# graphdeco-inria/hierarchical-3d-gaussians

Hardware: AMD Instinct MI355X
Metric: fwd+bwd frames/s @1080p, 1M Gaussians (higher is better)
Workload: dtype f32

## Files before the change

### hierarchical-3d-gaussians_amd/csrc/preprocess.hip

```cpp
#include "gaussian_math.h"

#include <stdlib.h>

#include <mutex>

namespace hgs {

namespace {

struct CamLds {
  float vm[16];
  float pm[16];
  float cam[3];
};

__device__ __forceinline__ void load_camera(const hgs_raster_args& a, CamLds& c) {
#pragma unroll
  for (int i = 0; i < 16; ++i) {
    c.vm[i] = a.viewmatrix[i];
    c.pm[i] = a.projmatrix[i];
  }
  c.cam[0] = a.campos[0];
  c.cam[1] = a.campos[1];
  c.cam[2] = a.campos[2];
// ... 747 lines not shown
}

constexpr int kPresumGrid = 2048;
__global__ __launch_bounds__(kPreBlock) void k8_presum_work_kernel(const uint2* __restrict__ work,
                                                                   const uint32_t* __restrict__ counter,
                                                                   const uint32_t* __restrict__ tiles_touched,
                                                                   const uint32_t* __restrict__ offsets,
                                                                   float* __restrict__ inst) {
  __shared__ double red_all[kPreBlock / 64][640 + 40];
  const int lane = threadIdx.x & 63, wave = threadIdx.x >> 6;
  const uint32_t n_work = *counter;
  double* red = red_all[wave];
  for (uint32_t item = blockIdx.x * (kPreBlock / 64) + wave; item < n_work; item += gridDim.x * (kPreBlock / 64)) {
    const uint2 w = work[item];
    const uint32_t n = tiles_touched[w.x];
    const uint32_t r0 = w.y * kK8Seg;
    const uint32_t r1 = (w.y + 1u == k8_nseg(n)) ? n : r0 + kK8Seg;
    const size_t rbase = (size_t)offsets[w.x] + r0;
    const float2* ip = reinterpret_cast<const float2*>(inst) + rbase * 5;
    double t[10];
#pragma unroll
    for (int i = 0; i < 10; ++i) t[i] = 0.0;
#pragma unroll 4
    for (uint32_t k = (uint32_t)lane; k < r1 - r0; k += 64u) {
      const float2 v0 = ip[k * 5 + 0], v1 = ip[k * 5 + 1], v2 = ip[k * 5 + 2], v3 = ip[k * 5 + 3], v4 = ip[k * 5 + 4];
      t[0] += v0.x; t[1] += v0.y; t[2] += v1.x; t[3] += v1.y;
      t[4] += v2.x; t[5] += v2.y; t[6] += v3.x; t[7] += v3.y;
      t[8] += v4.x; t[9] += v4.y;
    }
#pragma unroll
    for (int i = 0; i < 10; ++i) red[i * 64 + lane] = t[i];
    __builtin_amdgcn_fence(__ATOMIC_RELEASE, "wavefront");
    __builtin_amdgcn_wave_barrier();
    __builtin_amdgcn_fence(__ATOMIC_ACQUIRE, "wavefront");
    if (lane < 40) {
      double acc = 0.0;
      const double* src = red + (lane >> 2) * 64 + (lane & 3) * 16;
#pragma unroll
      for (int j = 0; j < 16; ++j) acc += src[j];
      red[640 + lane] = acc;
    }
    __builtin_amdgcn_fence(__ATOMIC_RELEASE, "wavefront");
    __builtin_amdgcn_wave_barrier();
    __builtin_amdgcn_fence(__ATOMIC_ACQUIRE, "wavefront");
    if (lane < 10) {
      const double* q = red + 640 + lane * 4;
      reinterpret_cast<double*>(inst + rbase * kInstStride)[lane] = ((q[0] + q[1]) + q[2]) + q[3];
    }
    __builtin_amdgcn_fence(__ATOMIC_RELEASE, "wavefront");
    __builtin_amdgcn_wave_barrier();
  }
}

template <bool ACC, bool LOD>
__global__ __launch_bounds__(kPreBlock) void preprocess_bwd_kernel(hgs_raster_args a, GeomWs g,
                                                                   const float* __restrict__ inst,
                                                                   float* __restrict__ drgb,
                                                                   float* __restrict__ dmean_rows,
                                                                   const uint32_t* __restrict__ lod_flag,
                                                                   hgs_raster_grads out, int presummed) {
  const int idx = blockIdx.x * kPreBlock + threadIdx.x;
  const bool in_range = idx < a.P;
  const uint32_t n = in_range ? g.tiles_touched[idx] : 0u;

  double s[10];
#pragma unroll
  for (int i = 0; i < 10; ++i) s[i] = 0.0;
  static_assert(kInstStride == 10, "instance record = the ten sums, 40 bytes");
  {
    constexpr uint32_t kStageRec = 256;
    __shared__ float2 stage[kPreBlock / 64][kStageRec * 5];
    const int lane = threadIdx.x & 63, wave = threadIdx.x >> 6;
    const unsigned long long long_mask = presummed ? __ballot(n > kK8LongRun) : 0ull;
    if (long_mask == 0ull) {
      uint32_t incl = n;
#pragma unroll
      for (int off = 1; off < 64; off <<= 1) {
        const uint32_t t = __shfl_up(incl, off, 64);
        if (lane >= off) incl += t;
      }
      const uint32_t my0 = incl - n, my1 = incl;
      const uint32_t total = __shfl(incl, 63, 64);
      if (total) {
        const unsigned long long nz = __ballot(n != 0u);
        const int first = __ffsll((long long)nz) - 1;
        const uint32_t off_mine = n ? g.offsets[idx] : 0u;
        const size_t base = (size_t)__shfl(off_mine, first, 64);
        float2* st = stage[wave];
        for (uint32_t c0 = 0; c0 < total; c0 += kStageRec) {
          const uint32_t cn = min(kStageRec, total - c0) * 5u;
          const float2* src = reinterpret_cast<const float2*>(inst) + (base + c0) * 5;
          for (uint32_t t0 = 0; t0 < cn; t0 += 64u * 4u) {
            float2 v[4];
#pragma unroll
            for (int j = 0; j < 4; ++j) {
              const uint32_t t = t0 + (uint32_t)j * 64u + (uint32_t)lane;
              v[j] = src[min(t, cn - 1u)];
            }
#pragma unroll
            for (int j = 0; j < 4; ++j) {
              const uint32_t t = t0 + (uint32_t)j * 64u + (uint32_t)lane;
              if (t < cn) st[t] = v[j];
            }
          }
          __builtin_amdgcn_fence(__ATOMIC_RELEASE, "wavefront");
          __builtin_amdgcn_wave_barrier();
          __builtin_amdgcn_fence(__ATOMIC_ACQUIRE, "wavefront");
          const uint32_t k0 = max(my0, c0), k1 = min(my1, c0 + kStageRec);
          for (uint32_t k = k0; k < k1; ++k) {
            const float2* r = st + (k - c0) * 5u;
            const float2 v0 = r[0], v1 = r[1], v2 = r[2], v3 = r[3], v4 = r[4];
            s[0] += v0.x; s[1] += v0.y; s[2] += v1.x; s[3] += v1.y;
            s[4] += v2.x; s[5] += v2.y; s[6] += v3.x; s[7] += v3.y;
            s[8] += v4.x; s[9] += v4.y;
          }
          __builtin_amdgcn_fence(__ATOMIC_RELEASE, "wavefront");
          __builtin_amdgcn_wave_barrier();
        }
      }
    } else if (n != 0u) {
      const size_t off = (size_t)g.offsets[idx];
      if (n > kK8LongRun) {
        const uint32_t nseg = k8_nseg(n);
        for (uint32_t j = 0; j < nseg; ++j) {
          const double* ps = reinterpret_cast<const double*>(inst + (off + (size_t)j * kK8Seg) * kInstStride);
#pragma unroll
          for (int i = 0; i < 10; ++i) s[i] += ps[i];
        }
      } else {
        const float2* ip = reinterpret_cast<const float2*>(inst) + off * 5;
#pragma unroll 2
        for (uint32_t k = 0; k < n; ++k) {
          const float2 v0 = ip[k * 5 + 0], v1 = ip[k * 5 + 1], v2 = ip[k * 5 + 2], v3 = ip[k * 5 + 3], v4 = ip[k * 5 + 4];
          s[0] += v0.x; s[1] += v0.y; s[2] += v1.x; s[3] += v1.y;
          s[4] += v2.x; s[5] += v2.y; s[6] += v3.x; s[7] += v3.y;
          s[8] += v4.x; s[9] += v4.y;
        }
      }
    }
  }
  if constexpr (!LOD) {
    if (!in_range) return;
  }

  float d_mean[3] = {0.f, 0.f, 0.f};
  float d_m2[3] = {0.f, 0.f, 0.f};
  float d_op = 0.f;
  float d_scale[3] = {0.f, 0.f, 0.f};
  float d_rot[4] = {0.f, 0.f, 0.f, 0.f};
  float d_c3[6] = {0.f, 0.f, 0.f, 0.f, 0.f, 0.f};
  float d_col[3] = {0.f, 0.f, 0.f};
  float sums6 = 0.f, sums7 = 0.f, sums8 = 0.f;

  if (n == 0) {
  } else {
    CamLds cam;
    load_camera(a, cam);
    sums6 = (float)s[6]; sums7 = (float)s[7]; sums8 = (float)s[8];
    const uint32_t flags = g.flags[idx];
    float p[3];
    load_mean<LOD>(a, lod_row_gather<LOD>(a, idx), p);
    float q[4] = {1.f, 0.f, 0.f, 0.f};
    float sc[3] = {1.f, 1.f, 1.f};
    double qnorm = 1.0;
    ProjD pd;
    if (a.cov3D_precomp) {
#pragma unroll
      for (int i = 0; i < 6; ++i) pd.c3[i] = (double)a.cov3D_precomp[(size_t)idx * 6 + i];
    } else {
      load_scale_rot<LOD>(a, idx, sc, q, &qnorm);
      cov3d_from_scale_rot_d(sc, a.scale_modifier, q, pd);
    }
    project_gaussian_d(p, cam.vm, cam.pm, a.width, a.height, a.tanfovx, a.tanfovy, (flags & 8u) != 0,
                       (flags & 16u) != 0, pd);

    const double A = pd.conA, B = pd.conB, C = pd.conC;
    const double gA = -0.5 * s[2], gB = -s[3], gC = -0.5 * s[4];
    const double ggx = -(A * s[0] + B * s[1]);
    const double ggy = -(C * s[1] + B * s[0]);
    const double dm2x = ggx * 0.5 * (double)a.width, dm2y = ggy * 0.5 * (double)a.height;
    d_m2[0] = (float)dm2x;
    d_m2[1] = (float)dm2y;
    double dmean[3] = {0.0, 0.0, 0.0};

    const double dhx = dm2x * pd.pw, dhy = dm2y * pd.pw;
    const double dhw = -(dm2x * pd.hx + dm2y * pd.hy) * pd.pw * pd.pw;
#pragma unroll
    for (int j = 0; j < 3; ++j)
      dmean[j] += (double)cam.pm[j * 4 + 0] * dhx + (double)cam.pm[j * 4 + 1] * dhy + (double)cam.pm[j * 4 + 3] * dhw;

    const double a2 = pd.a, b2 = pd.b, c2 = pd.c;
    const double di2 = pd.di * pd.di;
    const double ga = (-c2 * c2 * gA + b2 * c2 * gB - b2 * b2 * gC) * di2;
    const double gb = (2.0 * b2 * c2 * gA - (a2 * c2 + b2 * b2) * gB + 2.0 * a2 * b2 * gC) * di2;
    const double gc = (-b2 * b2 * gA + a2 * b2 * gB - a2 * a2 * gC) * di2;
    const double hb = 0.5 * gb;
    double Gs[3][3];
#pragma unroll
    for (int i = 0; i < 3; ++i)
#pragma unroll
      for (int j = i; j < 3; ++j)
        Gs[i][j] = Gs[j][i] = pd.T0[i] * (ga * pd.T0[j] + hb * pd.T1[j]) + pd.T1[i] * (hb * pd.T0[j] + gc * pd.T1[j]);
    d_c3[0] = (float)Gs[0][0];
    d_c3[1] = (float)(2.0 * Gs[0][1]);
    d_c3[2] = (float)(2.0 * Gs[0][2]);
    d_c3[3] = (float)Gs[1][1];
    d_c3[4] = (float)(2.0 * Gs[1][2]);
    d_c3[5] = (float)Gs[2][2];
    double dT0[3], dT1[3];
#pragma unroll
    for (int j = 0; j < 3; ++j) {
      dT0[j] = 2.0 * ga * pd.U0[j] + gb * pd.U1[j];
      dT1[j] = gb * pd.U0[j] + 2.0 * gc * pd.U1[j];
    }
    double gJ00 = 0.0, gJ02 = 0.0, gJ11 = 0.0, gJ12 = 0.0;
#pragma unroll
    for (int j = 0; j < 3; ++j) {
      gJ00 += dT0[j] * (double)cam.vm[j * 4 + 0];
      gJ02 += dT0[j] * (double)cam.vm[j * 4 + 2];
      gJ11 += dT1[j] * (double)cam.vm[j * 4 + 1];
      gJ12 += dT1[j] * (double)cam.vm[j * 4 + 2];
    }
    const double itz = pd.itz, itz2 = itz * itz, itz3 = itz2 * itz;
    const double g_txc = -pd.fx * itz2 * gJ02;
    const double g_tyc = -pd.fy * itz2 * gJ12;
    double g_tz = -pd.fx * itz2 * gJ00 + 2.0 * pd.fx * pd.txc * itz3 * gJ02 - pd.fy * itz2 * gJ11 +
                  2.0 * pd.fy * pd.tyc * itz3 * gJ12;
    double g_tx = 0.0, g_ty = 0.0;
    if (flags & 8u) g_tz += g_txc * (pd.txc * itz); else g_tx = g_txc;
    if (flags & 16u) g_tz += g_tyc * (pd.tyc * itz); else g_ty = g_tyc;
    g_tz += -s[9] * itz2;
#pragma unroll
    for (int j = 0; j < 3; ++j)
      dmean[j] += (double)cam.vm[j * 4 + 0] * g_tx + (double)cam.vm[j * 4 + 1] * g_ty + (double)cam.vm[j * 4 + 2] * g_tz;
    d_mean[0] = (float)dmean[0]; d_mean[1] = (float)dmean[1]; d_mean[2] = (float)dmean[2];

    if (!a.cov3D_precomp) {
      const double* R = pd.R;
      const double* sv = pd.s;
      double dM[3][3];
#pragma unroll
      for (int i = 0; i < 3; ++i)
#pragma unroll
        for (int k = 0; k < 3; ++k) {
          double acc = 0.0;
#pragma unroll
          for (int j = 0; j < 3; ++j) acc += Gs[i][j] * (R[j * 3 + k] * sv[k]);
          dM[i][k] = 2.0 * acc;
        }
      double gR[3][3];
#pragma unroll
      for (int k = 0; k < 3; ++k) {
        double acc = 0.0;
#pragma unroll
        for (int i = 0; i < 3; ++i) {
          acc += R[i * 3 + k] * dM[i][k];
          gR[i][k] = dM[i][k] * sv[k];
        }
        double dsk = (double)a.scale_modifier * acc;
        if (a.activations & HGS_ACT_SCALE_EXP) dsk *= (double)sc[k];
        d_scale[k] = (float)dsk;
      }
      const double r = q[0], x = q[1], y = q[2], z = q[3];
      double dq[4];
      dq[0] = 2.0 * (-z * gR[0][1] + y * gR[0][2] + z * gR[1][0] - x * gR[1][2] - y * gR[2][0] + x * gR[2][1]);
      dq[1] = 2.0 * (y * gR[0][1] + z * gR[0][2] + y * gR[1][0] - 2.0 * x * gR[1][1] - r * gR[1][2] +
                     z * gR[2][0] + r * gR[2][1] - 2.0 * x * gR[2][2]);
      dq[2] = 2.0 * (-2.0 * y * gR[0][0] + x * gR[0][1] + r * gR[0][2] + x * gR[1][0] + z * gR[1][2] -
                     r * gR[2][0] + z * gR[2][1] - 2.0 * y * gR[2][2]);
      dq[3] = 2.0 * (-2.0 * z * gR[0][0] - r * gR[0][1] + x * gR[0][2] + r * gR[1][0] - 2.0 * z * gR[1][1] +
                     y * gR[1][2] + x * gR[2][0] + y * gR[2][1]);
      if (a.activations & HGS_ACT_ROT_NORMALIZE) {
        const double dot = r * dq[0] + x * dq[1] + y * dq[2] + z * dq[3];
        const double inv = 1.0 / qnorm;
        dq[0] = (dq[0] - r * dot) * inv; dq[1] = (dq[1] - x * dot) * inv;
        dq[2] = (dq[2] - y * dot) * inv; dq[3] = (dq[3] - z * dot) * inv;
      }
      d_rot[0] = (float)dq[0]; d_rot[1] = (float)dq[1]; d_rot[2] = (float)dq[2]; d_rot[3] = (float)dq[3];
    }

    {
      float dod = 1.0f;
      double dact = 1.0;
      const float o_act = load_opacity<LOD>(a, idx, &dact);
      float o_rec = o_act;
      if (a.interpolation_weights && a.num_node_kids && !a.lod_per_pixel)
        o_rec = lod_opacity(o_act, a.interpolation_weights[idx], a.num_node_kids[idx], &dod);
      const float sums5 = o_rec > 0.0f ? (float)(s[5] / (double)o_rec) : 0.0f;
      d_op = a.activations ? (float)((double)sums5 * (double)dod * dact) : sums5 * dod;
    }

    float gr[3] = {sums6, sums7, sums8};
    if (a.colors_precomp) {
      d_col[0] = gr[0]; d_col[1] = gr[1]; d_col[2] = gr[2];
    } else {
      if (flags & 1u) gr[0] = 0.f;
      if (flags & 2u) gr[1] = 0.f;
      if (flags & 4u) gr[2] = 0.f;
      drgb[idx * 3 + 0] = gr[0];
      drgb[idx * 3 + 1] = gr[1];
      drgb[idx * 3 + 2] = gr[2];
    }
  }

  if constexpr (LOD) {
    if (a.lod_scatter) {
      __shared__ float lds_v[8 * kPreBlock];
      __shared__ int lds_par[kPreBlock];
      __shared__ unsigned char lds_vis[kPreBlock];
      const int t = threadIdx.x;
      const int block_first = blockIdx.x * kPreBlock;
      const int count = min(kPreBlock, a.P - block_first);
      LodRow l;
      l.r = l.p = 0; l.w = 1.0f; l.u = 0.0f;
      if (in_range) l = lod_row<true>(a, idx);
      const bool self = l.p == l.r;
      const bool vis = in_range && n != 0;
      const float wn = self ? 1.0f : l.w, u = (self || !vis) ? 0.0f : l.u;
      float sgn = 1.0f;
      if (vis && !self && u != 0.0f) {
        const float4 qa = reinterpret_cast<const float4*>(a.rotations)[l.r];
        const float4 qb = reinterpret_cast<const float4*>(a.rotations)[l.p];
        sgn = (qa.x * qb.x + qa.y * qb.y + qa.z * qb.z + qa.w * qb.w) < 0.0f ? -1.0f : 1.0f;
      }
      if (in_range) {
#pragma unroll
        for (int j = 0; j < 3; ++j) {
          dmean_rows[idx * 3 + j] = d_mean[j];
          out.dL_dmeans2D[idx * 3 + j] = d_m2[j];
        }
      }
      if (vis) {
        out.dL_dopacity[l.r] = wn * d_op;
#pragma unroll
        for (int j = 0; j < 3; ++j) out.dL_dscales[l.r * 3 + j] = wn * d_scale[j];
        reinterpret_cast<float4*>(out.dL_drotations)[l.r] = make_float4(wn * d_rot[0], wn * d_rot[1], wn * d_rot[2], wn * d_rot[3]);
      }
      lds_par[t] = in_range ? (int)l.p : -1;
      lds_vis[t] = (vis && !self) ? 1 : 0;
#pragma unroll
      for (int j = 0; j < 3; ++j) lds_v[j * kPreBlock + t] = u * d_scale[j];
#pragma unroll
      for (int j = 0; j < 4; ++j) lds_v[(3 + j) * kPreBlock + t] = (u * sgn) * d_rot[j];
      lds_v[7 * kPreBlock + t] = u * d_op;
      __syncthreads();
      if (t < count) {
        const LodRun run = lod_run(a, lds_par, t, count, block_first, *lod_flag != 0u);
        if (run.leader) {
          float acc8[8] = {0.f, 0.f, 0.f, 0.f, 0.f, 0.f, 0.f, 0.f};
          bool any = false;
          for (int j = t; j < run.end; ++j) {
            if (!lds_vis[j]) continue;
            any = true;
#pragma unroll
            for (int k = 0; k < 8; ++k) acc8[k] += lds_v[k * kPreBlock + j];
          }
          if (any) {
            const size_t pp = (size_t)lds_par[t];
#pragma unroll
            for (int k = 0; k < 3; ++k) lod_add(out.dL_dscales + pp * 3 + k, acc8[k], run.atomic);
#pragma unroll
            for (int k = 0; k < 4; ++k) lod_add(out.dL_drotations + pp * 4 + k, acc8[3 + k], run.atomic);
            lod_add(out.dL_dopacity + pp, acc8[7], run.atomic);
          }
        }
      }
      return;
    }
    if (!in_range) return;
  }
  constexpr bool acc = ACC;
#pragma unroll
  for (int j = 0; j < 3; ++j) {
    out.dL_dmeans3D[idx * 3 + j] = d_mean[j] + (acc ? out.dL_dmeans3D[idx * 3 + j] : 0.f);
    out.dL_dmeans2D[idx * 3 + j] = d_m2[j];
  }
  out.dL_dopacity[idx] = d_op + (acc ? out.dL_dopacity[idx] : 0.f);
  if (out.dL_dcolors) {
#pragma unroll
    for (int j = 0; j < 3; ++j) out.dL_dcolors[idx * 3 + j] = d_col[j];
  }
  if (out.dL_dscales) {
#pragma unroll
    for (int j = 0; j < 3; ++j) out.dL_dscales[idx * 3 + j] = d_scale[j] + (acc ? out.dL_dscales[idx * 3 + j] : 0.f);
  }
  if (out.dL_drotations) {
    float4* dst = reinterpret_cast<float4*>(out.dL_drotations) + idx;
    float4 v = make_float4(d_rot[0], d_rot[1], d_rot[2], d_rot[3]);
    if (acc) { const float4 o = *dst; v.x += o.x; v.y += o.y; v.z += o.z; v.w += o.w; }
    *dst = v;
  }
  if (out.dL_dcov3D) {
#pragma unroll
    for (int j = 0; j < 6; ++j) out.dL_dcov3D[(size_t)idx * 6 + j] = d_c3[j] + (acc ? out.dL_dcov3D[(size_t)idx * 6 + j] : 0.f);
  }
}


template <bool ACC, bool JAC, bool LOD>
__global__ __launch_bounds__(kPreBlock) void sh_bwd_kernel(hgs_raster_args a, GeomWs g,
                                                           const float* __restrict__ drgb,
                                                           const float* __restrict__ dmean_rows,
                                                           const uint32_t* __restrict__ lod_flag, hgs_raster_grads out) {
  extern __shared__ __attribute__((aligned(16))) unsigned char smem_raw[];
  float* lds = reinterpret_cast<float*>(smem_raw);
  const int n = a.M * 3;
  const bool split = a.shs_rest != nullptr;
  const bool coop = (n & 3) == 0;
  const int block_first = blockIdx.x * kPreBlock;
  const int idx = block_first + threadIdx.x;
  const bool valid = idx < a.P;
  const bool active = valid && g.tiles_touched[idx] != 0;
  if (!JAC && coop) {
    if (split) {
      coop_load_seg(a.shs, block_first, a.P, 3, 0, sh_row_stride(n), lds);
      coop_load_seg(a.shs_rest, block_first, a.P, n - 3, 3, sh_row_stride(n), lds);
    } else {
      coop_load_sh(a.shs, block_first, a.P, n, lds);
    }
    __syncthreads();
  }
  float dsh[48];
#pragma unroll
  for (int i = 0; i < 48; ++i) dsh[i] = 0.f;
  float sh[JAC ? 1 : 48];
  if constexpr (!JAC) {
    if (active) {
      if (coop) lds_row_read(lds, n, sh);
      else if (split) load_sh_split(a.shs, a.shs_rest, idx, a.M, sh);
      else load_sh(a.shs, idx, a.M, sh);
    }
  }
  if (!JAC && coop) __syncthreads();
  float vdir[3] = {0.f, 0.f, 0.f};
  if (active) {
    const float gr[3] = {drgb[idx * 3 + 0], drgb[idx * 3 + 1], drgb[idx * 3 + 2]};
    float pm[3];
    load_mean<LOD>(a, lod_row_gather<LOD>(a, idx), pm);
    float ux, uy, uz;
    const float inv = unit_dir(pm, a.campos, ux, uy, uz);
    float b[16];
    sh_basis(a.sh_degree, ux, uy, uz, b);
    const int nb = (a.sh_degree + 1) * (a.sh_degree + 1);
    float gdx = 0.f, gdy = 0.f, gdz = 0.f;
    if constexpr (JAC) {
      const float* jp = g.shjac + (size_t)idx * kJacStride;
      float J[9];
#pragma unroll
// ... 87 lines not shown
          const float wn = self ? 1.0f : rp[n + 2];
#pragma unroll
          for (int j = 0; j < 3; ++j) out.dL_dmeans3D[(size_t)r * 3 + j] = wn * lds_m[j * kPreBlock + t];
        }
        const LodRun run = lod_run(a, lds_par, t, count, block_first, nonmono);
        if (run.leader) {
          float acc3[3] = {0.f, 0.f, 0.f};
          bool any = false;
          for (int j = t; j < run.end; ++j) {
            const float* rj = lds + j * stride;
            if (!__float_as_uint(rj[n + 3]) || __float_as_uint(rj[n]) == __float_as_uint(rj[n + 1])) continue;
            any = true;
            const float uj = 1.0f - rj[n + 2];
#pragma unroll
            for (int k = 0; k < 3; ++k) acc3[k] += uj * lds_m[k * kPreBlock + j];
          }
          if (any) {
#pragma unroll
            for (int k = 0; k < 3; ++k) lod_add(out.dL_dmeans3D + (size_t)pr * 3 + k, acc3[k], run.atomic);
          }
        }
      }
      return;
    }
  }
  if (coop) {
    if (valid) lds_row_write(lds, n, dsh);
    __syncthreads();
    if (split) {
      coop_store_seg<ACC>(out.dL_dshs, block_first, a.P, 3, 0, sh_row_stride(n), lds);
      coop_store_seg<ACC>(out.dL_dshs_rest, block_first, a.P, n - 3, 3, sh_row_stride(n), lds);
    } else {
      coop_store_sh<ACC>(out.dL_dshs, block_first, a.P, n, lds);
    }
  } else if (valid && split) {
    float* d0 = out.dL_dshs + (size_t)idx * 3;
    float* d1 = out.dL_dshs_rest + (size_t)idx * (n - 3);
#pragma unroll
    for (int i = 0; i < 48; ++i) {
      if (i < 3) d0[i] = dsh[i] + (ACC ? d0[i] : 0.f);
      else if (i < n) d1[i - 3] = dsh[i] + (ACC ? d1[i - 3] : 0.f);
    }
  } else if (valid) {
    if (ACC) {
      const float* old = out.dL_dshs + (size_t)idx * n;
#pragma unroll
      for (int i = 0; i < 48; ++i)
        if (i < n) dsh[i] += old[i];
    }
    store_sh(out.dL_dshs, idx, a.M, dsh);
  }
}

template <bool ACC, bool COOP, bool COLOR>
__device__ __forceinline__ void sh_bwd_batched_body(const ShBwdViews& v, int P, int M, int sh_degree,
                                                    const float* __restrict__ means3D, const float* __restrict__ shs,
                                                    float* __restrict__ dL_dshs, float* __restrict__ dL_dmeans3D) {
  extern __shared__ __attribute__((aligned(16))) unsigned char smem_raw[];
  float* lds = reinterpret_cast<float*>(smem_raw);
  const int n = M * 3;
  constexpr bool coop = COOP;
  const int block_first = blockIdx.x * kPreBlock;
  const int idx = block_first + threadIdx.x;
  const bool valid = idx < P;
  if (coop) {
    coop_load_sh(shs, block_first, P, n, lds);
    __syncthreads();
  }
  float sh_reg[COOP ? 1 : 48];
  if constexpr (!COOP) { if (valid) load_sh(shs, idx, M, sh_reg); }
  float dsh[48];
#pragma unroll
  for (int i = 0; i < 48; ++i) dsh[i] = 0.f;
  float gm0 = 0.f, gm1 = 0.f, gm2 = 0.f;
  if (valid) {
    const float px = means3D[idx * 3 + 0], py = means3D[idx * 3 + 1], pz = means3D[idx * 3 + 2];
    const int nb = (sh_degree + 1) * (sh_degree + 1);
    for (int w = 0; w < v.n; ++w) {
      if (!COLOR && static_cast<const uint32_t*>(v.mask[w])[idx] == 0) continue;
      float gr0 = v.drgb[w][idx * 3 + 0], gr1 = v.drgb[w][idx * 3 + 1], gr2 = v.drgb[w][idx * 3 + 2];
      if (COLOR) {
        const uint32_t m = static_cast<const uint8_t*>(v.mask[w])[idx];
        if (m & 1u) gr0 = 0.f;
        if (m & 2u) gr1 = 0.f;
        if (m & 4u) gr2 = 0.f;
        if (gr0 == 0.f && gr1 == 0.f && gr2 == 0.f) continue;
      }
      float dotc[16];
#pragma unroll
      for (int k = 0; k < 16; ++k) dotc[k] = 0.f;
      if constexpr (COOP) {
        const float4* row4 = reinterpret_cast<const float4*>(lds + threadIdx.x * sh_row_stride(n));
#pragma unroll
        for (int i = 0; i < 12; ++i) {
          if (i * 4 < n) {
            const float4 t = row4[i];
            const float tv[4] = {t.x, t.y, t.z, t.w};
#pragma unroll
            for (int c = 0; c < 4; ++c) {
              const int ch = (i * 4 + c) % 3;
              dotc[(i * 4 + c) / 3] += (ch == 0 ? gr0 : ch == 1 ? gr1 : gr2) * tv[c];
            }
          }
        }
      } else {
#pragma unroll
// ... 198 lines not shown
  if (nblk > 0) {
    const bool jac = a.prepare_backward && a.shs;
    const bool plain = a.shs && !a.shs_rest && !a.lod_render_indices && ((a.M * 3) & 3) == 0;
    const bool h48 = plain && a.M == 16;
    const bool defer = plain && !h48;
    const size_t lds_bytes = !a.shs ? 0 : h48 ? (size_t)kK1ImageBytes : (size_t)kPreBlock * (a.M * 3 + 4) * sizeof(float);
    auto k1 = a.lod_render_indices ? (jac ? preprocess_fwd_kernel<true, true, false> : preprocess_fwd_kernel<false, true, false>)
              : h48   ? (jac ? preprocess_fwd_h48_kernel<true> : preprocess_fwd_h48_kernel<false>)
              : defer ? (jac ? preprocess_fwd_kernel<true, false, true> : preprocess_fwd_kernel<false, false, true>)
                      : (jac ? preprocess_fwd_kernel<true, false, false> : preprocess_fwd_kernel<false, false, false>);
    hipLaunchKernelGGL(k1, dim3(nblk), dim3(kPreBlock), lds_bytes, s, a, g, radii, super, heavy_thr);
    HGS_LAUNCH_CHECK("preprocess_fwd", s, a.debug);
  }
  return HGS_OK;
}

int launch_scan_block_sums(const GeomWs& g, int32_t P, hipStream_t s, bool debug, uint32_t* total_mirror) {
  const int nblk = (P + kPreBlock - 1) / kPreBlock;
  const int chunks = scan_chunks(nblk), resident = scan_resident_workgroups();
  if (chunks * (1 + kBands) <= resident && !scan_split_forced()) {
    hipLaunchKernelGGL(scan_block_sums_kernel, dim3(chunks, 1 + kBands), dim3(1024), 0, s, g.block_sums, g.block_band,
                       nblk, g.scan_chain, total_mirror, 0, chunks);
    HGS_LAUNCH_CHECK("scan_block_sums", s, debug);
    return HGS_OK;
  }
  for (int y = 0; y < 1 + kBands; ++y) {
    uint32_t* sums = y == 0 ? g.block_sums : g.block_band + (size_t)(y - 1) * (nblk + 1);
    for (int c0 = 0; c0 < chunks; c0 += resident) {
      hipLaunchKernelGGL(scan_block_sums_kernel, dim3(min(resident, chunks - c0), 1), dim3(1024), 0, s, sums, g.block_band,
                         nblk, g.scan_chain + (size_t)y * chunks, y == 0 ? total_mirror : nullptr, c0, chunks);
      HGS_LAUNCH_CHECK("scan_block_sums", s, debug);
    }
  }
  return HGS_OK;
}

int launch_preprocess_bwd(const hgs_raster_args& a, const GeomWs& g, const float* inst_grads, float* drgb,
                          float* dmean_rows, const uint32_t* lod_flag, const hgs_raster_grads& out, uint32_t L,
                          uint2* work, uint32_t* work_counter, hipStream_t s) {
  const int nblk = (a.P + kPreBlock - 1) / kPreBlock;
  if (nblk > 0) {
    static const char* force = getenv("HGS_K8_PRESUM");
    const bool presum = force ? force[0] == '1' : (uint64_t)L > 6ull * (uint64_t)a.P;
    if (presum) {
      HGS_HIP(hipMemsetAsync(work_counter, 0, sizeof(uint32_t), s));
      hipLaunchKernelGGL(k8_worklist_kernel, dim3(nblk < kWorklistGrid ? nblk : kWorklistGrid), dim3(kPreBlock), 0, s, a.P,
                         g.tiles_touched, work, work_counter);
      HGS_LAUNCH_CHECK("preprocess_bwd_worklist", s, a.debug);
      const int want = (int)(((size_t)L / 64 + 3) / 4);
      hipLaunchKernelGGL(k8_presum_work_kernel, dim3(want < 1 ? 1 : (want < kPresumGrid ? want : kPresumGrid)), dim3(kPreBlock), 0,
                         s, work, work_counter, g.tiles_touched, g.offsets, const_cast<float*>(inst_grads));
      HGS_LAUNCH_CHECK("preprocess_bwd_long_runs", s, a.debug);
    }
    auto k8a = a.lod_render_indices ? preprocess_bwd_kernel<false, true>
                                    : (a.accumulate_grads ? preprocess_bwd_kernel<true, false> : preprocess_bwd_kernel<false, false>);
    hipLaunchKernelGGL(k8a, dim3(nblk), dim3(kPreBlock), 0, s, a, g, inst_grads, drgb, dmean_rows, lod_flag, out,
                       presum ? 1 : 0);
    HGS_LAUNCH_CHECK("preprocess_bwd", s, a.debug);
    if (a.shs && out.dL_dshs && !a.defer_sh_bwd) {
      const size_t lds_bytes = (size_t)kPreBlock * (a.M * 3 + 4) * sizeof(float);
      auto k8b = a.lod_render_indices ? sh_bwd_kernel<false, true, true>
                 : (a.prepare_backward && a.shs) ? (a.accumulate_grads ? sh_bwd_kernel<true, true, false> : sh_bwd_kernel<false, true, false>)
                                                 : (a.accumulate_grads ? sh_bwd_kernel<true, false, false> : sh_bwd_kernel<false, false, false>);
      hipLaunchKernelGGL(k8b, dim3(nblk), dim3(kPreBlock), lds_bytes, s, a, g, drgb, dmean_rows, lod_flag, out);
      HGS_LAUNCH_CHECK("sh_bwd", s, a.debug);
    }
  }
  return HGS_OK;
}

}
```

Before: 1491.

## Fuse preprocess backward with SH backward into one kernel

Factors the per-Gaussian instance-sum reduction, gradient chain and row store into helpers. Adds a fused kernel that also does the SH backward in the same pass, using a precomputed SH Jacobian for the view-direction term on means. It stages dL/dSH rows through LDS for coalesced stores, reusing the staging buffer. This removes a second launch and the drgb/dmean round trip through global memory, at the cost of more registers and LDS per block, and only applies under a narrow set of flags.

Result: faster. 1537, median of 6 (+3.1%).

```diff
diff --git a/hierarchical-3d-gaussians_amd/csrc/preprocess.hip b/hierarchical-3d-gaussians_amd/csrc/preprocess.hip
--- a/hierarchical-3d-gaussians_amd/csrc/preprocess.hip
+++ b/hierarchical-3d-gaussians_amd/csrc/preprocess.hip
@@ -823,6 +823,252 @@
   }
 }
 
+constexpr uint32_t kK8StageRec = 256;
+__device__ __forceinline__ void k8_sum_runs(const GeomWs& g, const float* __restrict__ inst, int idx, uint32_t n,
+                                            int presummed, float2* st, double (&s)[10]) {
+  const int lane = threadIdx.x & 63;
+  const unsigned long long long_mask = presummed ? __ballot(n > kK8LongRun) : 0ull;
+  if (long_mask == 0ull) {
+    uint32_t incl = n;
+#pragma unroll
+    for (int off = 1; off < 64; off <<= 1) {
+      const uint32_t t = __shfl_up(incl, off, 64);
+      if (lane >= off) incl += t;
+    }
+    const uint32_t my0 = incl - n, my1 = incl;
+    const uint32_t total = __shfl(incl, 63, 64);
+    if (total) {
+      const unsigned long long nz = __ballot(n != 0u);
+      const int first = __ffsll((long long)nz) - 1;
+      const uint32_t off_mine = n ? g.offsets[idx] : 0u;
+      const size_t base = (size_t)__shfl(off_mine, first, 64);
+      for (uint32_t c0 = 0; c0 < total; c0 += kK8StageRec) {
+        const uint32_t cn = min(kK8StageRec, total - c0) * 5u;
+        const float2* src = reinterpret_cast<const float2*>(inst) + (base + c0) * 5;
+        for (uint32_t t0 = 0; t0 < cn; t0 += 64u * 4u) {
+          float2 v[4];
+#pragma unroll
+          for (int j = 0; j < 4; ++j) {
+            const uint32_t t = t0 + (uint32_t)j * 64u + (uint32_t)lane;
+            v[j] = src[min(t, cn - 1u)];
+          }
+#pragma unroll
+          for (int j = 0; j < 4; ++j) {
+            const uint32_t t = t0 + (uint32_t)j * 64u + (uint32_t)lane;
+            if (t < cn) st[t] = v[j];
+          }
+        }
+        __builtin_amdgcn_fence(__ATOMIC_RELEASE, "wavefront");
+        __builtin_amdgcn_wave_barrier();
+        __builtin_amdgcn_fence(__ATOMIC_ACQUIRE, "wavefront");
+        const uint32_t k0 = max(my0, c0), k1 = min(my1, c0 + kK8StageRec);
+        for (uint32_t k = k0; k < k1; ++k) {
+          const float2* r = st + (k - c0) * 5u;
+          const float2 v0 = r[0], v1 = r[1], v2 = r[2], v3 = r[3], v4 = r[4];
+          s[0] += v0.x; s[1] += v0.y; s[2] += v1.x; s[3] += v1.y;
+          s[4] += v2.x; s[5] += v2.y; s[6] += v3.x; s[7] += v3.y;
+          s[8] += v4.x; s[9] += v4.y;
+        }
+        __builtin_amdgcn_fence(__ATOMIC_RELEASE, "wavefront");
+        __builtin_amdgcn_wave_barrier();
+      }
+    }
+  } else if (n != 0u) {
+    const size_t off = (size_t)g.offsets[idx];
+    if (n > kK8LongRun) {
+      const uint32_t nseg = k8_nseg(n);
+      for (uint32_t j = 0; j < nseg; ++j) {
+        const double* ps = reinterpret_cast<const double*>(inst + (off + (size_t)j * kK8Seg) * kInstStride);
+#pragma unroll
+        for (int i = 0; i < 10; ++i) s[i] += ps[i];
+      }
+    } else {
+      const float2* ip = reinterpret_cast<const float2*>(inst) + off * 5;
+#pragma unroll 2
+      for (uint32_t k = 0; k < n; ++k) {
+        const float2 v0 = ip[k * 5 + 0], v1 = ip[k * 5 + 1], v2 = ip[k * 5 + 2], v3 = ip[k * 5 + 3], v4 = ip[k * 5 + 4];
+        s[0] += v0.x; s[1] += v0.y; s[2] += v1.x; s[3] += v1.y;
+        s[4] += v2.x; s[5] += v2.y; s[6] += v3.x; s[7] += v3.y;
+        s[8] += v4.x; s[9] += v4.y;
+      }
+    }
+  }
+}
+
+template <bool LOD>
+__device__ __forceinline__ void k8_chain(const hgs_raster_args& a, const GeomWs& g, int idx, const double (&s)[10],
+                                         float (&p)[3], float (&d_mean)[3], float (&d_m2)[3], float& d_op,
+                                         float (&d_scale)[3], float (&d_rot)[4], float (&d_c3)[6], float (&gr)[3]) {
+  CamLds cam;
+  load_camera(a, cam);
+  gr[0] = (float)s[6]; gr[1] = (float)s[7]; gr[2] = (float)s[8];
+  const uint32_t flags = g.flags[idx];
+  load_mean<LOD>(a, lod_row_gather<LOD>(a, idx), p);
+  float q[4] = {1.f, 0.f, 0.f, 0.f};
+  float sc[3] = {1.f, 1.f, 1.f};
+  double qnorm = 1.0;
+  ProjD pd;
+  if (a.cov3D_precomp) {
+#pragma unroll
+    for (int i = 0; i < 6; ++i) pd.c3[i] = (double)a.cov3D_precomp[(size_t)idx * 6 + i];
+  } else {
+    load_scale_rot<LOD>(a, idx, sc, q, &qnorm);
+    cov3d_from_scale_rot_d(sc, a.scale_modifier, q, pd);
+  }
+  project_gaussian_d(p, cam.vm, cam.pm, a.width, a.height, a.tanfovx, a.tanfovy, (flags & 8u) != 0,
+                     (flags & 16u) != 0, pd);
+
+  const double A = pd.conA, B = pd.conB, C = pd.conC;
+  const double gA = -0.5 * s[2], gB = -s[3], gC = -0.5 * s[4];
+  const double ggx = -(A * s[0] + B * s[1]);
+  const double ggy = -(C * s[1] + B * s[0]);
+  const double dm2x = ggx * 0.5 * (double)a.width, dm2y = ggy * 0.5 * (double)a.height;
+  d_m2[0] = (float)dm2x;
+  d_m2[1] = (float)dm2y;
+  double dmean[3] = {0.0, 0.0, 0.0};
+
+  const double dhx = dm2x * pd.pw, dhy = dm2y * pd.pw;
+  const double dhw = -(dm2x * pd.hx + dm2y * pd.hy) * pd.pw * pd.pw;
+#pragma unroll
+  for (int j = 0; j < 3; ++j)
+    dmean[j] += (double)cam.pm[j * 4 + 0] * dhx + (double)cam.pm[j * 4 + 1] * dhy + (double)cam.pm[j * 4 + 3] * dhw;
+
+  const double a2 = pd.a, b2 = pd.b, c2 = pd.c;
+  const double di2 = pd.di * pd.di;
+  const double ga = (-c2 * c2 * gA + b2 * c2 * gB - b2 * b2 * gC) * di2;
+  const double gb = (2.0 * b2 * c2 * gA - (a2 * c2 + b2 * b2) * gB + 2.0 * a2 * b2 * gC) * di2;
+  const double gc = (-b2 * b2 * gA + a2 * b2 * gB - a2 * a2 * gC) * di2;
+  const double hb = 0.5 * gb;
+  double Gs[3][3];
+#pragma unroll
+  for (int i = 0; i < 3; ++i)
+#pragma unroll
+    for (int j = i; j < 3; ++j)
+      Gs[i][j] = Gs[j][i] = pd.T0[i] * (ga * pd.T0[j] + hb * pd.T1[j]) + pd.T1[i] * (hb * pd.T0[j] + gc * pd.T1[j]);
+  d_c3[0] = (float)Gs[0][0];
+  d_c3[1] = (float)(2.0 * Gs[0][1]);
+  d_c3[2] = (float)(2.0 * Gs[0][2]);
+  d_c3[3] = (float)Gs[1][1];
+  d_c3[4] = (float)(2.0 * Gs[1][2]);
+  d_c3[5] = (float)Gs[2][2];
+  double dT0[3], dT1[3];
+#pragma unroll
+  for (int j = 0; j < 3; ++j) {
+    dT0[j] = 2.0 * ga * pd.U0[j] + gb * pd.U1[j];
+    dT1[j] = gb * pd.U0[j] + 2.0 * gc * pd.U1[j];
+  }
+  double gJ00 = 0.0, gJ02 = 0.0, gJ11 = 0.0, gJ12 = 0.0;
+#pragma unroll
+  for (int j = 0; j < 3; ++j) {
+    gJ00 += dT0[j] * (double)cam.vm[j * 4 + 0];
+    gJ02 += dT0[j] * (double)cam.vm[j * 4 + 2];
+    gJ11 += dT1[j] * (double)cam.vm[j * 4 + 1];
+    gJ12 += dT1[j] * (double)cam.vm[j * 4 + 2];
+  }
+  const double itz = pd.itz, itz2 = itz * itz, itz3 = itz2 * itz;
+  const double g_txc = -pd.fx * itz2 * gJ02;
+  const double g_tyc = -pd.fy * itz2 * gJ12;
+  double g_tz = -pd.fx * itz2 * gJ00 + 2.0 * pd.fx * pd.txc * itz3 * gJ02 - pd.fy * itz2 * gJ11 +
+                2.0 * pd.fy * pd.tyc * itz3 * gJ12;
+  double g_tx = 0.0, g_ty = 0.0;
+  if (flags & 8u) g_tz += g_txc * (pd.txc * itz); else g_tx = g_txc;
+  if (flags & 16u) g_tz += g_tyc * (pd.tyc * itz); else g_ty = g_tyc;
+  g_tz += -s[9] * itz2;
+#pragma unroll
+  for (int j = 0; j < 3; ++j)
+    dmean[j] += (double)cam.vm[j * 4 + 0] * g_tx + (double)cam.vm[j * 4 + 1] * g_ty + (double)cam.vm[j * 4 + 2] * g_tz;
+  d_mean[0] = (float)dmean[0]; d_mean[1] = (float)dmean[1]; d_mean[2] = (float)dmean[2];
+
+  if (!a.cov3D_precomp) {
+    const double* R = pd.R;
+    const double* sv = pd.s;
+    double dM[3][3];
+#pragma unroll
+    for (int i = 0; i < 3; ++i)
+#pragma unroll
+      for (int k = 0; k < 3; ++k) {
+        double acc = 0.0;
+#pragma unroll
+        for (int j = 0; j < 3; ++j) acc += Gs[i][j] * (R[j * 3 + k] * sv[k]);
+        dM[i][k] = 2.0 * acc;
+      }
+    double gR[3][3];
+#pragma unroll
+    for (int k = 0; k < 3; ++k) {
+      double acc = 0.0;
+#pragma unroll
+      for (int i = 0; i < 3; ++i) {
+        acc += R[i * 3 + k] * dM[i][k];
+        gR[i][k] = dM[i][k] * sv[k];
+      }
+      double dsk = (double)a.scale_modifier * acc;
+      if (a.activations & HGS_ACT_SCALE_EXP) dsk *= (double)sc[k];
+      d_scale[k] = (float)dsk;
+    }
+    const double r = q[0], x = q[1], y = q[2], z = q[3];
+    double dq[4];
+    dq[0] = 2.0 * (-z * gR[0][1] + y * gR[0][2] + z * gR[1][0] - x * gR[1][2] - y * gR[2][0] + x * gR[2][1]);
+    dq[1] = 2.0 * (y * gR[0][1] + z * gR[0][2] + y * gR[1][0] - 2.0 * x * gR[1][1] - r * gR[1][2] +
+                   z * gR[2][0] + r * gR[2][1] - 2.0 * x * gR[2][2]);
+    dq[2] = 2.0 * (-2.0 * y * gR[0][0] + x * gR[0][1] + r * gR[0][2] + x * gR[1][0] + z * gR[1][2] -
+                   r * gR[2][0] + z * gR[2][1] - 2.0 * y * gR[2][2]);
+    dq[3] = 2.0 * (-2.0 * z * gR[0][0] - r * gR[0][1] + x * gR[0][2] + r * gR[1][0] - 2.0 * z * gR[1][1] +
+                   y * gR[1][2] + x * gR[2][0] + y * gR[2][1]);
+    if (a.activations & HGS_ACT_ROT_NORMALIZE) {
+      const double dot = r * dq[0] + x * dq[1] + y * dq[2] + z * dq[3];
+      const double inv = 1.0 / qnorm;
+      dq[0] = (dq[0] - r * dot) * inv; dq[1] = (dq[1] - x * dot) * inv;
+      dq[2] = (dq[2] - y * dot) * inv; dq[3] = (dq[3] - z * dot) * inv;
+    }
+    d_rot[0] = (float)dq[0]; d_rot[1] = (float)dq[1]; d_rot[2] = (float)dq[2]; d_rot[3] = (float)dq[3];
+  }
+
+  {
+    float dod = 1.0f;
+    double dact = 1.0;
+    const float o_act = load_opacity<LOD>(a, idx, &dact);
+    float o_rec = o_act;
+    if (a.interpolation_weights && a.num_node_kids && !a.lod_per_pixel)
+      o_rec = lod_opacity(o_act, a.interpolation_weights[idx], a.num_node_kids[idx], &dod);
+    const float sums5 = o_rec > 0.0f ? (float)(s[5] / (double)o_rec) : 0.0f;
+    d_op = a.activations ? (float)((double)sums5 * (double)dod * dact) : sums5 * dod;
+  }
+
+  if (!a.colors_precomp) {
+    if (flags & 1u) gr[0] = 0.f;
+    if (flags & 2u) gr[1] = 0.f;
+    if (flags & 4u) gr[2] = 0.f;
+  }
+}
+
+template <bool ACC>
+__device__ __forceinline__ void k8_store_row(const hgs_raster_grads& out, int idx, const float (&d_m2)[3], float d_op,
+                                             const float (&d_scale)[3], const float (&d_rot)[4], const float (&d_c3)[6],
+                                             const float (&d_col)[3]) {
+  constexpr bool acc = ACC;
+#pragma unroll
+  for (int j = 0; j < 3; ++j) out.dL_dmeans2D[idx * 3 + j] = d_m2[j];
+  out.dL_dopacity[idx] = d_op + (acc ? out.dL_dopacity[idx] : 0.f);
+  if (out.dL_dcolors) {
+#pragma unroll
+    for (int j = 0; j < 3; ++j) out.dL_dcolors[idx * 3 + j] = d_col[j];
+  }
+  if (out.dL_dscales) {
+#pragma unroll
+    for (int j = 0; j < 3; ++j) out.dL_dscales[idx * 3 + j] = d_scale[j] + (acc ? out.dL_dscales[idx * 3 + j] : 0.f);
+  }
+  if (out.dL_drotations) {
+    float4* dst = reinterpret_cast<float4*>(out.dL_drotations) + idx;
+    float4 v = make_float4(d_rot[0], d_rot[1], d_rot[2], d_rot[3]);
+    if (acc) { const float4 o = *dst; v.x += o.x; v.y += o.y; v.z += o.z; v.w += o.w; }
+    *dst = v;
+  }
+  if (out.dL_dcov3D) {
+#pragma unroll
+    for (int j = 0; j < 6; ++j) out.dL_dcov3D[(size_t)idx * 6 + j] = d_c3[j] + (acc ? out.dL_dcov3D[(size_t)idx * 6 + j] : 0.f);
+  }
+}
+
 template <bool ACC, bool LOD>
 __global__ __launch_bounds__(kPreBlock) void preprocess_bwd_kernel(hgs_raster_args a, GeomWs g,
                                                                    const float* __restrict__ inst,
@@ -838,78 +1084,8 @@
 #pragma unroll
   for (int i = 0; i < 10; ++i) s[i] = 0.0;
   static_assert(kInstStride == 10, "instance record = the ten sums, 40 bytes");
-  {
-    constexpr uint32_t kStageRec = 256;
-    __shared__ float2 stage[kPreBlock / 64][kStageRec * 5];
-    const int lane = threadIdx.x & 63, wave = threadIdx.x >> 6;
-    const unsigned long long long_mask = presummed ? __ballot(n > kK8LongRun) : 0ull;
-    if (long_mask == 0ull) {
-      uint32_t incl = n;
-#pragma unroll
-      for (int off = 1; off < 64; off <<= 1) {
-        const uint32_t t = __shfl_up(incl, off, 64);
-        if (lane >= off) incl += t;
-      }
-      const uint32_t my0 = incl - n, my1 = incl;
-      const uint32_t total = __shfl(incl, 63, 64);
-      if (total) {
-        const unsigned long long nz = __ballot(n != 0u);
-        const int first = __ffsll((long long)nz) - 1;
-        const uint32_t off_mine = n ? g.offsets[idx] : 0u;
-        const size_t base = (size_t)__shfl(off_mine, first, 64);
-        float2* st = stage[wave];
-        for (uint32_t c0 = 0; c0 < total; c0 += kStageRec) {
-          const uint32_t cn = min(kStageRec, total - c0) * 5u;
-          const float2* src = reinterpret_cast<const float2*>(inst) + (base + c0) * 5;
-          for (uint32_t t0 = 0; t0 < cn; t0 += 64u * 4u) {
-            float2 v[4];
-#pragma unroll
-            for (int j = 0; j < 4; ++j) {
-              const uint32_t t = t0 + (uint32_t)j * 64u + (uint32_t)lane;
-              v[j] = src[min(t, cn - 1u)];
-            }
-#pragma unroll
-            for (int j = 0; j < 4; ++j) {
-              const uint32_t t = t0 + (uint32_t)j * 64u + (uint32_t)lane;
-              if (t < cn) st[t] = v[j];
-            }
-          }
-          __builtin_amdgcn_fence(__ATOMIC_RELEASE, "wavefront");
-          __builtin_amdgcn_wave_barrier();
-          __builtin_amdgcn_fence(__ATOMIC_ACQUIRE, "wavefront");
-          const uint32_t k0 = max(my0, c0), k1 = min(my1, c0 + kStageRec);
-          for (uint32_t k = k0; k < k1; ++k) {
-            const float2* r = st + (k - c0) * 5u;
-            const float2 v0 = r[0], v1 = r[1], v2 = r[2], v3 = r[3], v4 = r[4];
-            s[0] += v0.x; s[1] += v0.y; s[2] += v1.x; s[3] += v1.y;
-            s[4] += v2.x; s[5] += v2.y; s[6] += v3.x; s[7] += v3.y;
-            s[8] += v4.x; s[9] += v4.y;
-          }
-          __builtin_amdgcn_fence(__ATOMIC_RELEASE, "wavefront");
-          __builtin_amdgcn_wave_barrier();
-        }
-      }
-    } else if (n != 0u) {
-      const size_t off = (size_t)g.offsets[idx];
-      if (n > kK8LongRun) {
-        const uint32_t nseg = k8_nseg(n);
-        for (uint32_t j = 0; j < nseg; ++j) {
-          const double* ps = reinterpret_cast<const double*>(inst + (off + (size_t)j * kK8Seg) * kInstStride);
-#pragma unroll
-          for (int i = 0; i < 10; ++i) s[i] += ps[i];
-        }
-      } else {
-        const float2* ip = reinterpret_cast<const float2*>(inst) + off * 5;
-#pragma unroll 2
-        for (uint32_t k = 0; k < n; ++k) {
-          const float2 v0 = ip[k * 5 + 0], v1 = ip[k * 5 + 1], v2 = ip[k * 5 + 2], v3 = ip[k * 5 + 3], v4 = ip[k * 5 + 4];
-          s[0] += v0.x; s[1] += v0.y; s[2] += v1.x; s[3] += v1.y;
-          s[4] += v2.x; s[5] += v2.y; s[6] += v3.x; s[7] += v3.y;
-          s[8] += v4.x; s[9] += v4.y;
-        }
-      }
-    }
-  }
+  __shared__ float2 stage[kPreBlock / 64][kK8StageRec * 5];
+  k8_sum_runs(g, inst, idx, n, presummed, stage[threadIdx.x >> 6], s);
   if constexpr (!LOD) {
     if (!in_range) return;
   }
@@ -920,154 +1096,14 @@
   float d_scale[3] = {0.f, 0.f, 0.f};
   float d_rot[4] = {0.f, 0.f, 0.f, 0.f};
   float d_c3[6] = {0.f, 0.f, 0.f, 0.f, 0.f, 0.f};
+  float gr[3] = {0.f, 0.f, 0.f};
   float d_col[3] = {0.f, 0.f, 0.f};
-  float sums6 = 0.f, sums7 = 0.f, sums8 = 0.f;
-
-  if (n == 0) {
-  } else {
-    CamLds cam;
-    load_camera(a, cam);
-    sums6 = (float)s[6]; sums7 = (float)s[7]; sums8 = (float)s[8];
-    const uint32_t flags = g.flags[idx];
+  if (n != 0) {
     float p[3];
-    load_mean<LOD>(a, lod_row_gather<LOD>(a, idx), p);
-    float q[4] = {1.f, 0.f, 0.f, 0.f};
-    float sc[3] = {1.f, 1.f, 1.f};
-    double qnorm = 1.0;
-    ProjD pd;
-    if (a.cov3D_precomp) {
-#pragma unroll
-      for (int i = 0; i < 6; ++i) pd.c3[i] = (double)a.cov3D_precomp[(size_t)idx * 6 + i];
-    } else {
-      load_scale_rot<LOD>(a, idx, sc, q, &qnorm);
-      cov3d_from_scale_rot_d(sc, a.scale_modifier, q, pd);
-    }
-    project_gaussian_d(p, cam.vm, cam.pm, a.width, a.height, a.tanfovx, a.tanfovy, (flags & 8u) != 0,
-                       (flags & 16u) != 0, pd);
-
-    const double A = pd.conA, B = pd.conB, C = pd.conC;
-    const double gA = -0.5 * s[2], gB = -s[3], gC = -0.5 * s[4];
-    const double ggx = -(A * s[0] + B * s[1]);
-    const double ggy = -(C * s[1] + B * s[0]);
-    const double dm2x = ggx * 0.5 * (double)a.width, dm2y = ggy * 0.5 * (double)a.height;
-    d_m2[0] = (float)dm2x;
-    d_m2[1] = (float)dm2y;
-    double dmean[3] = {0.0, 0.0, 0.0};
-
-    const double dhx = dm2x * pd.pw, dhy = dm2y * pd.pw;
-    const double dhw = -(dm2x * pd.hx + dm2y * pd.hy) * pd.pw * pd.pw;
-#pragma unroll
-    for (int j = 0; j < 3; ++j)
-      dmean[j] += (double)cam.pm[j * 4 + 0] * dhx + (double)cam.pm[j * 4 + 1] * dhy + (double)cam.pm[j * 4 + 3] * dhw;
-
-    const double a2 = pd.a, b2 = pd.b, c2 = pd.c;
-    const double di2 = pd.di * pd.di;
-    const double ga = (-c2 * c2 * gA + b2 * c2 * gB - b2 * b2 * gC) * di2;
-    const double gb = (2.0 * b2 * c2 * gA - (a2 * c2 + b2 * b2) * gB + 2.0 * a2 * b2 * gC) * di2;
-    const double gc = (-b2 * b2 * gA + a2 * b2 * gB - a2 * a2 * gC) * di2;
-    const double hb = 0.5 * gb;
-    double Gs[3][3];
-#pragma unroll
-    for (int i = 0; i < 3; ++i)
-#pragma unroll
-      for (int j = i; j < 3; ++j)
-        Gs[i][j] = Gs[j][i] = pd.T0[i] * (ga * pd.T0[j] + hb * pd.T1[j]) + pd.T1[i] * (hb * pd.T0[j] + gc * pd.T1[j]);
-    d_c3[0] = (float)Gs[0][0];
-    d_c3[1] = (float)(2.0 * Gs[0][1]);
-    d_c3[2] = (float)(2.0 * Gs[0][2]);
-    d_c3[3] = (float)Gs[1][1];
-    d_c3[4] = (float)(2.0 * Gs[1][2]);
-    d_c3[5] = (float)Gs[2][2];
-    double dT0[3], dT1[3];
-#pragma unroll
-    for (int j = 0; j < 3; ++j) {
-      dT0[j] = 2.0 * ga * pd.U0[j] + gb * pd.U1[j];
-      dT1[j] = gb * pd.U0[j] + 2.0 * gc * pd.U1[j];
-    }
-    double gJ00 = 0.0, gJ02 = 0.0, gJ11 = 0.0, gJ12 = 0.0;
-#pragma unroll
-    for (int j = 0; j < 3; ++j) {
-      gJ00 += dT0[j] * (double)cam.vm[j * 4 + 0];
-      gJ02 += dT0[j] * (double)cam.vm[j * 4 + 2];
-      gJ11 += dT1[j] * (double)cam.vm[j * 4 + 1];
-      gJ12 += dT1[j] * (double)cam.vm[j * 4 + 2];
-    }
-    const double itz = pd.itz, itz2 = itz * itz, itz3 = itz2 * itz;
-    const double g_txc = -pd.fx * itz2 * gJ02;
-    const double g_tyc = -pd.fy * itz2 * gJ12;
-    double g_tz = -pd.fx * itz2 * gJ00 + 2.0 * pd.fx * pd.txc * itz3 * gJ02 - pd.fy * itz2 * gJ11 +
-                  2.0 * pd.fy * pd.tyc * itz3 * gJ12;
-    double g_tx = 0.0, g_ty = 0.0;
-    if (flags & 8u) g_tz += g_txc * (pd.txc * itz); else g_tx = g_txc;
-    if (flags & 16u) g_tz += g_tyc * (pd.tyc * itz); else g_ty = g_tyc;
-    g_tz += -s[9] * itz2;
-#pragma unroll
-    for (int j = 0; j < 3; ++j)
-      dmean[j] += (double)cam.vm[j * 4 + 0] * g_tx + (double)cam.vm[j * 4 + 1] * g_ty + (double)cam.vm[j * 4 + 2] * g_tz;
-    d_mean[0] = (float)dmean[0]; d_mean[1] = (float)dmean[1]; d_mean[2] = (float)dmean[2];
-
-    if (!a.cov3D_precomp) {
-      const double* R = pd.R;
-      const double* sv = pd.s;
-      double dM[3][3];
-#pragma unroll
-      for (int i = 0; i < 3; ++i)
-#pragma unroll
-        for (int k = 0; k < 3; ++k) {
-          double acc = 0.0;
-#pragma unroll
-          for (int j = 0; j < 3; ++j) acc += Gs[i][j] * (R[j * 3 + k] * sv[k]);
-          dM[i][k] = 2.0 * acc;
-        }
-      double gR[3][3];
-#pragma unroll
-      for (int k = 0; k < 3; ++k) {
-        double acc = 0.0;
-#pragma unroll
-        for (int i = 0; i < 3; ++i) {
-          acc += R[i * 3 + k] * dM[i][k];
-          gR[i][k] = dM[i][k] * sv[k];
-        }
-        double dsk = (double)a.scale_modifier * acc;
-        if (a.activations & HGS_ACT_SCALE_EXP) dsk *= (double)sc[k];
-        d_scale[k] = (float)dsk;
-      }
-      const double r = q[0], x = q[1], y = q[2], z = q[3];
-      double dq[4];
-      dq[0] = 2.0 * (-z * gR[0][1] + y * gR[0][2] + z * gR[1][0] - x * gR[1][2] - y * gR[2][0] + x * gR[2][1]);
-      dq[1] = 2.0 * (y * gR[0][1] + z * gR[0][2] + y * gR[1][0] - 2.0 * x * gR[1][1] - r * gR[1][2] +
-                     z * gR[2][0] + r * gR[2][1] - 2.0 * x * gR[2][2]);
-      dq[2] = 2.0 * (-2.0 * y * gR[0][0] + x * gR[0][1] + r * gR[0][2] + x * gR[1][0] + z * gR[1][2] -
-                     r * gR[2][0] + z * gR[2][1] - 2.0 * y * gR[2][2]);
-      dq[3] = 2.0 * (-2.0 * z * gR[0][0] - r * gR[0][1] + x * gR[0][2] + r * gR[1][0] - 2.0 * z * gR[1][1] +
-                     y * gR[1][2] + x * gR[2][0] + y * gR[2][1]);
-      if (a.activations & HGS_ACT_ROT_NORMALIZE) {
-        const double dot = r * dq[0] + x * dq[1] + y * dq[2] + z * dq[3];
-        const double inv = 1.0 / qnorm;
-        dq[0] = (dq[0] - r * dot) * inv; dq[1] = (dq[1] - x * dot) * inv;
-        dq[2] = (dq[2] - y * dot) * inv; dq[3] = (dq[3] - z * dot) * inv;
-      }
-      d_rot[0] = (float)dq[0]; d_rot[1] = (float)dq[1]; d_rot[2] = (float)dq[2]; d_rot[3] = (float)dq[3];
-    }
-
-    {
-      float dod = 1.0f;
-      double dact = 1.0;
-      const float o_act = load_opacity<LOD>(a, idx, &dact);
-      float o_rec = o_act;
-      if (a.interpolation_weights && a.num_node_kids && !a.lod_per_pixel)
-        o_rec = lod_opacity(o_act, a.interpolation_weights[idx], a.num_node_kids[idx], &dod);
-      const float sums5 = o_rec > 0.0f ? (float)(s[5] / (double)o_rec) : 0.0f;
-      d_op = a.activations ? (float)((double)sums5 * (double)dod * dact) : sums5 * dod;
-    }
-
-    float gr[3] = {sums6, sums7, sums8};
+    k8_chain<LOD>(a, g, idx, s, p, d_mean, d_m2, d_op, d_scale, d_rot, d_c3, gr);
     if (a.colors_precomp) {
       d_col[0] = gr[0]; d_col[1] = gr[1]; d_col[2] = gr[2];
     } else {
-      if (flags & 1u) gr[0] = 0.f;
-      if (flags & 2u) gr[1] = 0.f;
-      if (flags & 4u) gr[2] = 0.f;
       drgb[idx * 3 + 0] = gr[0];
       drgb[idx * 3 + 1] = gr[1];
       drgb[idx * 3 + 2] = gr[2];
@@ -1140,31 +1176,9 @@
     }
     if (!in_range) return;
   }
-  constexpr bool acc = ACC;
-#pragma unroll
-  for (int j = 0; j < 3; ++j) {
-    out.dL_dmeans3D[idx * 3 + j] = d_mean[j] + (acc ? out.dL_dmeans3D[idx * 3 + j] : 0.f);
-    out.dL_dmeans2D[idx * 3 + j] = d_m2[j];
-  }
-  out.dL_dopacity[idx] = d_op + (acc ? out.dL_dopacity[idx] : 0.f);
-  if (out.dL_dcolors) {
-#pragma unroll
-    for (int j = 0; j < 3; ++j) out.dL_dcolors[idx * 3 + j] = d_col[j];
-  }
-  if (out.dL_dscales) {
-#pragma unroll
-    for (int j = 0; j < 3; ++j) out.dL_dscales[idx * 3 + j] = d_scale[j] + (acc ? out.dL_dscales[idx * 3 + j] : 0.f);
-  }
-  if (out.dL_drotations) {
-    float4* dst = reinterpret_cast<float4*>(out.dL_drotations) + idx;
-    float4 v = make_float4(d_rot[0], d_rot[1], d_rot[2], d_rot[3]);
-    if (acc) { const float4 o = *dst; v.x += o.x; v.y += o.y; v.z += o.z; v.w += o.w; }
-    *dst = v;
-  }
-  if (out.dL_dcov3D) {
-#pragma unroll
-    for (int j = 0; j < 6; ++j) out.dL_dcov3D[(size_t)idx * 6 + j] = d_c3[j] + (acc ? out.dL_dcov3D[(size_t)idx * 6 + j] : 0.f);
-  }
+#pragma unroll
+  for (int j = 0; j < 3; ++j) out.dL_dmeans3D[idx * 3 + j] = d_mean[j] + (ACC ? out.dL_dmeans3D[idx * 3 + j] : 0.f);
+  k8_store_row<ACC>(out, idx, d_m2, d_op, d_scale, d_rot, d_c3, d_col);
 }
 
 
@@ -1358,6 +1372,92 @@
   }
 }
 
+__device__ __forceinline__ float k8_dot3(float x0, float y0, float x1, float y1, float x2, float y2) {
+#pragma clang fp contract(off)
+  return __fmaf_rn(x2, y2, __fmaf_rn(x0, y0, x1 * y1));
+}
+__device__ __forceinline__ void k8_add_view_term(const float (&gr)[3], const float (&J)[9], float ux, float uy, float uz,
+                                                 float inv, float (&d_mean)[3]) {
+#pragma clang fp contract(off)
+  const float gdx = k8_dot3(gr[0], J[0], gr[1], J[1], gr[2], J[2]);
+  const float gdy = k8_dot3(gr[0], J[3], gr[1], J[4], gr[2], J[5]);
+  const float gdz = k8_dot3(gr[0], J[6], gr[1], J[7], gr[2], J[8]);
+  const float dot = k8_dot3(ux, gdx, uy, gdy, uz, gdz);
+  d_mean[0] = __fmaf_rn(__fmaf_rn(-ux, dot, gdx), inv, d_mean[0] + 0.f);
+  d_mean[1] = __fmaf_rn(__fmaf_rn(-uy, dot, gdy), inv, d_mean[1] + 0.f);
+  d_mean[2] = __fmaf_rn(__fmaf_rn(-uz, dot, gdz), inv, d_mean[2] + 0.f);
+}
+
+__global__ __launch_bounds__(kPreBlock) void preprocess_bwd_sh_kernel(hgs_raster_args a, GeomWs g,
+                                                                         const float* __restrict__ inst,
+                                                                         hgs_raster_grads out, int presummed) {
+  extern __shared__ __attribute__((aligned(16))) unsigned char smem_raw[];
+  const int block_first = blockIdx.x * kPreBlock;
+  const int idx = block_first + threadIdx.x;
+  const bool in_range = idx < a.P;
+  const uint32_t n = in_range ? g.tiles_touched[idx] : 0u;
+
+  double s[10];
+#pragma unroll
+  for (int i = 0; i < 10; ++i) s[i] = 0.0;
+  k8_sum_runs(g, inst, idx, n, presummed, reinterpret_cast<float2*>(smem_raw) + (threadIdx.x >> 6) * (kK8StageRec * 5), s);
+
+  float d_mean[3] = {0.f, 0.f, 0.f};
+  float d_m2[3] = {0.f, 0.f, 0.f};
+  float d_op = 0.f;
+  float d_scale[3] = {0.f, 0.f, 0.f};
+  float d_rot[4] = {0.f, 0.f, 0.f, 0.f};
+  float d_c3[6] = {0.f, 0.f, 0.f, 0.f, 0.f, 0.f};
+  float gr[3] = {0.f, 0.f, 0.f};
+  float b[16];
+  const int nb = (a.sh_degree + 1) * (a.sh_degree + 1);
+  float p[3];
+  if (n != 0) k8_chain<false>(a, g, idx, s, p, d_mean, d_m2, d_op, d_scale, d_rot, d_c3, gr);
+  if (in_range) {
+    const float d_col[3] = {0.f, 0.f, 0.f};
+    k8_store_row<false>(out, idx, d_m2, d_op, d_scale, d_rot, d_c3, d_col);
+  }
+  __builtin_amdgcn_sched_barrier(0);
+  if (n != 0) {
+    float ux, uy, uz;
+    const float inv = unit_dir(p, a.campos, ux, uy, uz);
+    sh_basis(a.sh_degree, ux, uy, uz, b);
+    const float* jp = g.shjac + (size_t)idx * kJacStride;
+    float J[9];
+#pragma unroll
+    for (int k = 0; k < 9; ++k) J[k] = jp[k];
+    k8_add_view_term(gr, J, ux, uy, uz, inv, d_mean);
+  } else {
+#pragma unroll
+    for (int j = 0; j < 3; ++j) d_mean[j] = 0.f;
+  }
+  if (in_range) {
+#pragma unroll
+    for (int j = 0; j < 3; ++j) out.dL_dmeans3D[idx * 3 + j] = d_mean[j];
+  }
+
+  float* lds = reinterpret_cast<float*>(smem_raw);
+  const int nc = a.M * 3, stride = sh_row_stride(nc);
+  __syncthreads();
+  if (in_range) {
+    float* row = lds + threadIdx.x * stride;
+#pragma unroll
+    for (int i = 0; i < 12; ++i) {
+      if (i * 4 < nc) {
+        float v[4];
+#pragma unroll
+        for (int c = 0; c < 4; ++c) {
+          const int k = (i * 4 + c) / 3, ch = (i * 4 + c) % 3;
+          v[c] = (n != 0 && k < nb) ? b[k] * gr[ch] : 0.f;
+        }
+        *reinterpret_cast<float4*>(row + i * 4) = make_float4(v[0], v[1], v[2], v[3]);
+      }
+    }
+  }
+  __syncthreads();
+  coop_store_sh<false>(out.dL_dshs, block_first, a.P, nc, lds);
+}
+
 template <bool ACC, bool COOP, bool COLOR>
 __device__ __forceinline__ void sh_bwd_batched_body(const ShBwdViews& v, int P, int M, int sh_degree,
                                                     const float* __restrict__ means3D, const float* __restrict__ shs,
@@ -1662,6 +1762,18 @@
                          s, work, work_counter, g.tiles_touched, g.offsets, const_cast<float*>(inst_grads));
       HGS_LAUNCH_CHECK("preprocess_bwd_long_runs", s, a.debug);
     }
+    const char* fuse_env = getenv("HGS_K8_FUSE");
+    const bool fused = !(fuse_env && fuse_env[0] == '0') && !a.lod_render_indices && !a.accumulate_grads &&
+                       !a.defer_sh_bwd && a.shs && !a.shs_rest && out.dL_dshs && a.prepare_backward && !a.colors_precomp &&
+                       ((a.M * 3) & 3) == 0;
+    if (fused) {
+      const size_t stage_bytes = (size_t)(kPreBlock / 64) * kK8StageRec * 5 * sizeof(float2);
+      const size_t rows_bytes = (size_t)kPreBlock * (a.M * 3 + 4) * sizeof(float);
+      hipLaunchKernelGGL(preprocess_bwd_sh_kernel, dim3(nblk), dim3(kPreBlock),
+                         stage_bytes > rows_bytes ? stage_bytes : rows_bytes, s, a, g, inst_grads, out, presum ? 1 : 0);
+      HGS_LAUNCH_CHECK("preprocess_bwd_sh", s, a.debug);
+      return HGS_OK;
+    }
     auto k8a = a.lod_render_indices ? preprocess_bwd_kernel<false, true>
                                     : (a.accumulate_grads ? preprocess_bwd_kernel<true, false> : preprocess_bwd_kernel<false, false>);
     hipLaunchKernelGGL(k8a, dim3(nblk), dim3(kPreBlock), 0, s, a, g, inst_grads, drgb, dmean_rows, lod_flag, out,
```
